# tanksha/das

Hardware: AMD Instinct MI355X
Metric: pattern matches/sec (bindings/s) + % HBM roofline (higher is better)
Workload: dtype u32; 1 GPU; config2 bio gene-level KB (+ annotation layouts): single-Link + 2-clause And (Q1-Q4) + scripts/benchmark.py QUERY_1-3 (Q3, Q5, Q6); parallelism=links sharded x1, step_calls=matched() per query

## Files before the change

das_amd/csrc/das_internal.h:

```cpp
#pragma once
#include <array>
#include <atomic>
#include <map>
#include <unordered_map>
#include <memory>
#include <mutex>
#include <string>
#include <vector>

#include "../../include/das_mi355x.h"
#include "common.h"
#include "prims.h"

namespace das {

constexpr int kMaxArity = 8;
constexpr int kMaxPosArity = 3;
constexpr int kMaxCols = 16;
constexpr int kTypeBits = 24;

enum AtomCat : uint8_t { CAT_OTHER = 0, CAT_NODE = 1, CAT_LINK = 2, CAT_LINK_REMOTE = 3 };
enum CatPrio : uint8_t { PRIO_OTHER = 0, PRIO_NODE = 1, PRIO_REMOTE = 2, PRIO_LINK = 3 };
__host__ __device__ inline uint8_t cat_of_prio(uint32_t p) {
  return p == PRIO_LINK ? CAT_LINK : p == PRIO_REMOTE ? CAT_LINK_REMOTE : p == PRIO_NODE ? CAT_NODE : CAT_OTHER;
// ... 46 lines not shown
struct Index {
  bool built = false;
  hipStream_t stream = nullptr;
  uint64_t n_atoms = 0, n_nodes = 0, n_links = 0, n_types = 0;
  uint32_t shard_world = 1;
  Digest* digest = nullptr;
  uint32_t* by_digest = nullptr;
  uint8_t* cat = nullptr;
  uint32_t* type = nullptr;
  uint32_t* arity = nullptr;
  uint64_t* tgt_off = nullptr;
  uint32_t* in_off = nullptr;
  uint32_t* in_link = nullptr;
  uint64_t in_total = 0;
  uint32_t* tgt = nullptr;
  uint32_t* ctype = nullptr;
  uint32_t* name_leaf = nullptr;
  std::array<RowTable, kMaxArity + 1> ttab{};
  std::array<RowTable, kMaxArity + 1> ctab{};
  std::array<std::array<PosIndex, kMaxPosArity>, kMaxPosArity + 1> pidx{};
  std::array<std::vector<uint64_t>, kMaxArity + 1> type_off;
  std::array<std::vector<uint32_t>, kMaxArity + 1> tbound, gbound;
  std::vector<Digest> ctype_digest;
  std::vector<Digest> type_digest;
  std::vector<uint8_t> no_pattern;
  bool no_pattern_any = false;
  bool blocked(uint32_t ty) const { return ty < no_pattern.size() && no_pattern[ty]; }
  std::vector<uint32_t> type_name_len;
  std::vector<CtypeRange> ctype_range;
  std::vector<Digest> h_node_dig;
  std::vector<uint32_t> h_node_id, h_node_type;
  NameHeap names;
  std::vector<void*> owned;
  std::map<std::array<uint64_t, 4>, std::pair<uint64_t, uint64_t>> range_cache;
  uint64_t device_bytes = 0;
};

struct Ctx;
struct Table;

struct Expansion;
struct ExpansionDel {
  void operator()(Expansion* e) const;
};

struct Lazy {
  enum Kind : uint8_t { PRODUCT = 0, VIEW = 1, EXPAND = 2 };
  Kind kind = PRODUCT;
  Ctx* ctx = nullptr;
  Table* owner = nullptr;
  std::atomic<bool> listed{false};
  std::unique_ptr<Expansion, ExpansionDel> exp;
  bool aliases_index() const { return kind != PRODUCT; }
  uint32_t* buf = nullptr;
  uint64_t np = 0, nb = 0, pcap = 0, bcap = 0;
  int ncp = 0, ncb = 0;
  int32_t pvars[kMaxCols] = {0}, bvars[kMaxCols] = {0};
  uint8_t side[kMaxCols] = {0}, src[kMaxCols] = {0};
  const uint32_t* pcol(int k) const { return buf + (uint64_t)k * pcap; }
  const uint32_t* bcol(int k) const { return buf + (uint64_t)ncp * pcap + (uint64_t)k * bcap; }
  Lazy() = default;
  Lazy(const Lazy&) = delete;
  Lazy& operator=(const Lazy&) = delete;
  ~Lazy() {
    if (buf) cache_free(buf);
  }
};

struct Table {
  int kind = DAS_TABLE_ORDERED;
  int ncols = 0;
  int sorted_col = -1;
  int32_t vars[kMaxCols] = {0};
  int32_t member[kMaxCols] = {0};
  uint32_t lo[kMaxCols] = {0};
  uint32_t hi[kMaxCols] = {kNone, kNone, kNone, kNone, kNone, kNone, kNone, kNone,
                           kNone, kNone, kNone, kNone, kNone, kNone, kNone, kNone};
  uint64_t nrows = 0, cap = 0;
  uint32_t* data = nullptr;
  hipStream_t s = nullptr;
  bool view = false;
  std::shared_ptr<Lazy> lazy;
  uint32_t* col(int c) const {
    DAS_CHECK(!lazy, DAS_E_INTERNAL, "column of an unresolved table");
    return data + (uint64_t)c * cap;
  }
  ~Table() {
    if (data && !view) cache_free(data);
  }
};

struct KStat {
  double ms = 0, bytes = 0;
  uint64_t launches = 0;
};
struct PendingEv {
  std::string name;
  hipEvent_t a, b;
  double bytes;
};

struct Ctx {
  bool prof = false;
  int scan_views = 0;
  std::string prof_only;
  std::string prof_tag;
  uint32_t tag_plan = ~0u;
  std::string tag_plan_name;
  hipStream_t gate_s = nullptr;
  double gate_min = 0;
  bool prof_selected(const std::string& name) const {
    if (prof_only.empty()) return true;
    size_t b = 0;
    while (b <= prof_only.size()) {
      size_t e = prof_only.find('|', b);
      if (e == std::string::npos) e = prof_only.size();
      if (prof_only.compare(b, e - b, name) == 0) return true;
      b = e + 1;
// ... 125 lines not shown
void partition_rows(Ctx& c, const uint32_t* d_rows, uint64_t n, uint32_t K, const uint8_t* d_owner, uint32_t world,
                    uint32_t* d_out, uint64_t* counts);
void numbered_strings(const char* prefix, uint64_t plen, uint64_t first, uint64_t n, uint8_t* out, uint64_t* off);
void synth_powerlaw_links(uint32_t* d_child, uint64_t first, uint64_t n, uint32_t K, uint32_t n_link_types,
                          uint32_t type_leaf0, uint32_t node_leaf0, uint64_t n_nodes, double s, uint64_t seed,
                          hipStream_t st);
void free_index(Ctx& c);
void lookup_digests(Ctx& c, const Digest* h_digests, uint64_t n, int64_t* h_ids);
bool lookup_small(Ctx& c, const Digest* h_digests, uint64_t n, int64_t* h_ids, uint8_t* cat, uint32_t* arity,
                  uint32_t* type);

void ensure_name_heap(Ctx& c);
void check_name_dfa(const das_name_dfa_t& d);
uint64_t match_node_names(Ctx& c, uint32_t type_id, const das_name_dfa_t& d, uint32_t* out_ids, uint64_t cap);
std::unique_ptr<struct Table> scan_node_names(Ctx& c, uint32_t type_id, const das_name_dfa_t& d, int32_t var);
std::unique_ptr<struct Table> table_name_filter(Ctx& c, const struct Table& t, int32_t var, uint32_t type_id,
                                                const das_name_dfa_t& d, int mode);
uint64_t node_names(Ctx& c, const uint32_t* h_ids, const uint32_t* d_ids, uint64_t n, uint64_t* off, uint8_t* bytes,
                    uint64_t cap, uint8_t* kind, uint64_t* n_other);

uint64_t atoms_json(Ctx& c, const uint32_t* h_ids, const uint32_t* d_ids, uint64_t n, uint32_t as_list,
                    const uint8_t* type_json, const uint64_t* type_json_off, uint32_t n_types, uint8_t* out,
                    uint64_t cap, uint64_t* n_other, uint64_t* n_bad_utf8);
uint64_t links_outgoing(Ctx& c, const uint32_t* h_ids, const uint32_t* d_ids, uint64_t n, uint64_t* off,
                        uint32_t* targets, uint64_t cap, uint32_t* ctype, uint8_t* kind);

void halo_expand(Ctx& c, const uint32_t* seed_ids, uint64_t n_seeds, uint32_t levels,
                 std::vector<std::unique_ptr<Table>>& links, std::vector<std::unique_ptr<Table>>& atoms);
std::unique_ptr<Table> pattern_counts(Ctx& c, const uint32_t* d_links, uint64_t n);
void conjunction_counts(Ctx& c, const uint32_t* tpl, uint64_t m, const uint32_t* combo, uint64_t n, uint32_t k,
                        uint64_t* counts);
void mine_combinations(Ctx& c, const uint32_t* tpl, uint64_t m, const uint64_t* tpl_count, const uint32_t* basics,
                       uint64_t nb, const uint32_t* cands, uint64_t nc, uint32_t k, uint64_t universe_size,
                       uint64_t support, bool normalized, uint32_t top, uint64_t max_combinations,
                       uint32_t* out_combo, uint64_t* out_count, double* out_value, uint32_t* n_out,
                       uint64_t stats[3]);

struct ColSet {
  const uint32_t* c[kMaxCols];
  int n;
};

ColSet cols_of(const Table& t);
void sort_perm(const ColSet& cs, uint64_t n, uint32_t* perm, int bits, hipStream_t s);
int id_bits(const Ctx& c);
std::unique_ptr<Table> gather_table(Ctx& c, const Table& a, const uint32_t* idx, uint64_t m);
std::unique_ptr<Table> gather_ranges(Ctx& c, const Table& a, const uint64_t* begin, const uint64_t* end,
                                     uint32_t n_ranges);
std::unique_ptr<Table> compact_table(Ctx& c, const Table& a, const uint32_t* keep);
void join_ranges(Ctx& c, const ColSet& probe, uint64_t np, const ColSet& build_sorted, uint64_t nb, uint32_t* lo,
                 uint32_t* cnt);
std::unique_ptr<Table> scan_link(Ctx& c, const das_link_scan_t& q);
std::unique_ptr<Table> scan_template(Ctx& c, const das_template_scan_t& q);
std::unique_ptr<Table> join(Ctx& c, const Table& a, const Table& b, int flags, bool defer_product = false);
void settle(Ctx& c, Table& t);
void register_alias(Table& t);
void deregister_alias(Lazy& r);
void settle_aliases(Ctx& c);
bool defer_join_rows(uint64_t probe_rows, uint64_t out_rows);
void make_lazy_view(Ctx& c, Table& t);
std::unique_ptr<Table> product_rows(Ctx& c, const Table& t, uint64_t row0, uint64_t n);
struct ExpansionCol {
  const uint32_t* key = nullptr;
  const uint32_t* rowid = nullptr;
  const uint2* lc = nullptr;
  uint64_t n = 0;
};
bool expansion_probe_col(const Table& t, int col, ExpansionCol& out);
void product_checksum(Ctx& c, const Table& t, const uint64_t* salt, uint64_t out[2]);
std::unique_ptr<Table> semi_join_multi(Ctx& c, const Table& p, const std::vector<const Table*>& qs);
std::unique_ptr<Table> index_join_filtered(Ctx& c, const Table& a, const das_link_scan_t& q, int32_t fvar,
                                           const std::vector<const Table*>& qs);
std::unique_ptr<Table> index_join(Ctx& c, const Table& a, const das_link_scan_t& q,
                                  std::unique_ptr<Table>* take = nullptr);
std::unique_ptr<Table> anti_index_join(Ctx& c, const Table& a, const das_link_scan_t& q);
std::unique_ptr<Table> antijoin(Ctx& c, const Table& a, const Table& t);
std::unique_ptr<Table> dedup(Ctx& c, const Table& a);
std::unique_ptr<Table> concat(Ctx& c, const Table* const* ts, int n);
std::unique_ptr<Table> new_table(Ctx& c, int kind, int ncols, const int32_t* vars, uint64_t cap,
                                 const int32_t* member = nullptr);
inline std::unique_ptr<Table> new_table_like(Ctx& c, const Table& a, uint64_t cap) {
  auto t = new_table(c, a.kind, a.ncols, a.vars, cap, a.member);
  t->sorted_col = a.sorted_col;
  for (int k = 0; k < a.ncols; ++k) {
    t->lo[k] = a.lo[k];
    t->hi[k] = a.hi[k];
  }
  return t;
}
std::unique_ptr<Table> partition(Ctx& c, const Table& t, const int32_t* key_vars, uint32_t nkey, uint32_t nparts,
                                 uint64_t* counts);
void export_rows(Ctx& c, const Table& t, uint32_t* dst);
void table_checksum(Ctx& c, const Table& t, const uint64_t* salt, uint64_t out[2]);
double box_store_bw(Ctx& c, uint64_t bytes, uint32_t reps);
void prof_mark(Ctx& c, uint32_t id);
std::unique_ptr<Table> import_rows(Ctx& c, int kind, int ncols, const int32_t* vars, const int32_t* member,
                                   const uint32_t* src, uint64_t n);

struct PlanOutput {
  bool matched = false, negation = false;
  std::vector<std::unique_ptr<Table>> tables;
};
PlanOutput plan_execute(Ctx& c, const das_plan_node_t* nodes, uint32_t n, int no_overload);
std::vector<PlanOutput> plan_execute_many(Ctx& c, const das_plan_node_t* const* nodes, const uint32_t* n,
                                          uint32_t n_plans, int no_overload);
PlanOutput plan_execute_sharded(Ctx& c, const das_plan_node_t* nodes, uint32_t n, int no_overload,
                                const std::vector<const Table*>& inputs, std::vector<uint8_t>& checks);
// ... 48 lines not shown
```

das_amd/csrc/plan.hip:

```cpp
#include <functional>
#include <memory>
#include <vector>

#include "das_internal.h"

namespace das {
namespace {

using TablePtr = std::unique_ptr<Table>;

struct Rel {
  std::vector<TablePtr> t;
  bool partial = false;
  bool nonempty() const {
    for (auto& x : t)
      if (x->nrows) return true;
    return false;
  }
  void push(TablePtr x) {
    if (x && x->nrows) t.push_back(std::move(x));
  }
};

struct Res {
// ... 26 lines not shown
  uint32_t next(uint32_t i) const {
    DAS_CHECK(i < n, DAS_E_INVALID, "plan: truncated node array");
    const das_plan_node_t& x = nd[i];
    if (x.op == DAS_PLAN_LINK || x.op == DAS_PLAN_CONST || x.op == DAS_PLAN_INPUT || x.op == DAS_PLAN_TEMPLATE)
      return i + 1;
    if (x.op == DAS_PLAN_NOT) return next(i + 1);
    DAS_CHECK(x.op == DAS_PLAN_AND || x.op == DAS_PLAN_OR || x.op == DAS_PLAN_TVM, DAS_E_INVALID,
              "plan: bad node op");
    uint32_t j = i + 1;
    for (uint32_t k = 0; k < x.nchild; ++k) j = next(j);
    return j;
  }

  std::vector<uint32_t> children(uint32_t i) const {
    std::vector<uint32_t> out;
    uint32_t j = i + 1;
    for (uint32_t k = 0; k < nd[i].nchild; ++k) {
      out.push_back(j);
      j = next(j);
    }
    return out;
  }

  Rel normalize(Rel a) {
    std::vector<std::vector<TablePtr>> groups;
    for (auto& x : a.t) {
      bool put = false;
      for (auto& g : groups)
        if (same_schema(*g[0], *x)) {
          g.push_back(std::move(x));
          put = true;
          break;
        }
      if (!put) {
        groups.emplace_back();
        groups.back().push_back(std::move(x));
      }
    }
    Rel out;
    out.partial = a.partial;
    for (auto& g : groups) {
      if (g.size() == 1) {
        out.push(std::move(g[0]));
        continue;
      }
      std::vector<const Table*> ts;
      for (auto& x : g) ts.push_back(x.get());
      auto cat = concat(c, ts.data(), (int)ts.size());
      out.push(dedup(c, *cat));
    }
    return out;
  }

  Rel join_rel(const Rel& a, const Rel& b, bool defer = false) {
    Rel out;
    out.partial = a.partial || b.partial;
    for (auto& ta : a.t)
      for (auto& tb : b.t) out.push(join(c, *ta, *tb, no_overload, defer && defer_rows(ta->nrows, tb->nrows)));
    return out;
  }

  static bool defer_rows(uint64_t na, uint64_t nb) {
    const char f = env_char("DAS_DEFER_PRODUCT");
    if (f == '0') return false;
    return f == '1' || na * nb > (1ull << 20);
  }

  void settle_for_normalize(Rel& acc) {
    for (size_t i = 0; i < acc.t.size(); ++i) {
      if (!acc.t[i]->lazy) continue;
      for (size_t j = 0; j < acc.t.size(); ++j)
        if (j != i && same_schema(*acc.t[i], *acc.t[j])) {
          settle(c, *acc.t[i]);
          break;
        }
    }
  }

  Rel antijoin_rel(Rel r, const Rel& f) {
    for (auto& ft : f.t) {
      Rel nx;
      nx.partial = r.partial;
      for (auto& t : r.t) nx.push(antijoin(c, *t, *ft));
      r = std::move(nx);
    }
    return r;
  }

  Rel minus_rel(Rel a, const Rel& b) {
    Rel out;
    out.partial = a.partial;
    for (auto& t : a.t) {
      TablePtr cur = std::move(t);
      for (auto& f : b.t)
        if (cur && cur->nrows && same_schema(*cur, *f)) cur = antijoin(c, *cur, *f);
      out.push(std::move(cur));
    }
    return out;
  }

  Res eval(uint32_t i) {
    const das_plan_node_t& x = nd[i];
    static const char* const kOp[] = {"?", "LINK", "CONST", "NOT", "AND", "OR", "INPUT", "TEMPLATE", "TVM"};
    if (trace_on()) trace_mark("node", x.op <= 8 ? kOp[x.op] : "?");
    Res r;
    switch (x.op) {
      case DAS_PLAN_CONST:
        r.matched = x.value != 0;
        return r;
      case DAS_PLAN_LINK: {
        DAS_CHECK(x.scan.ordered, DAS_E_UNSUPPORTED, "plan: unordered Link terms take the host path");
// ... 625 lines not shown
```

das_amd/csrc/query.hip:

```cpp
#include <algorithm>
#include <cstddef>
#include <cstdlib>
#include <cstring>
#include <optional>
#include <string>
#include <type_traits>

#include "das_internal.h"

namespace das {

namespace {

struct FlagIn {
  const uint32_t* a;
  uint64_t n;
  __device__ uint32_t operator()(uint64_t i) const { return i < n ? a[i] : 0u; }
};

struct WidenCnt {
  const uint32_t* a;
  uint64_t n;
  __device__ uint64_t operator()(uint64_t i) const { return i < n ? (uint64_t)a[i] : 0ull; }
};

constexpr unsigned B = 256;
constexpr int kChunkIters = 16;
constexpr uint64_t kChunk = (uint64_t)B * kChunkIters;
inline dim3 G(uint64_t n) { return dim3(grid_for(n, B)); }

struct ScanSpec {
  const uint32_t* col[kMaxArity + 1];
  uint32_t arity;
  uint32_t fixed[kMaxArity];
  int32_t outpos[kMaxCols];
  uint32_t nout;
  uint32_t eq_a[kMaxArity], eq_b[kMaxArity], neq;
  uint32_t no_overload;
  uint32_t unordered;
  uint32_t upos[kMaxArity], nupos;
  uint32_t emit_link;
  uint32_t all_keep;
};

__device__ __forceinline__ bool scan_keep(const ScanSpec& sp, uint64_t r) {
  if (sp.all_keep) return true;
  for (uint32_t p = 0; p < sp.arity; ++p)
    if (sp.fixed[p] != kNone && sp.col[1 + p][r] != sp.fixed[p]) return false;
  for (uint32_t e = 0; e < sp.neq; ++e)
    if (sp.col[1 + sp.eq_a[e]][r] != sp.col[1 + sp.eq_b[e]][r]) return false;
  if (sp.unordered) {
    for (uint32_t i = 0; i < sp.nupos; ++i)
      for (uint32_t j = i + 1; j < sp.nupos; ++j)
        if (sp.col[1 + sp.upos[i]][r] == sp.col[1 + sp.upos[j]][r]) return false;
  } else if (sp.no_overload) {
    const uint32_t base = sp.emit_link ? 1 : 0;
    for (uint32_t i = base; i < sp.nout; ++i)
      for (uint32_t j = i + 1; j < sp.nout; ++j)
        if (sp.col[1 + sp.outpos[i]][r] == sp.col[1 + sp.outpos[j]][r]) return false;
  }
  return true;
// ... 1382 lines not shown
std::unique_ptr<Table> gather_ranges(Ctx& c, const Table& a, const uint64_t* begin, const uint64_t* end,
                                     uint32_t n_ranges) {
  std::vector<uint64_t> h(2 * (uint64_t)n_ranges + 1, 0);
  uint64_t m = 0, last = 0;
  bool ascending = true;
  for (uint32_t i = 0; i < n_ranges; ++i) {
    DAS_CHECK(begin[i] <= end[i] && end[i] <= a.nrows, DAS_E_INVALID, "gather range outside the table");
    h[i] = m;
    h[n_ranges + 1 + i] = begin[i];
    m += end[i] - begin[i];
    if (end[i] > begin[i]) {
      if (begin[i] < last) ascending = false;
      last = end[i] - 1;
    }
  }
  h[n_ranges] = m;
  auto t = new_table_like(c, a, m);
  t->nrows = m;
  if (!ascending) t->sorted_col = -1;
  if (m && a.ncols) {
    DBuf<uint64_t> d(h.size(), c.s);
    DAS_HIP(hipMemcpyAsync(d.p, h.data(), 8 * h.size(), hipMemcpyHostToDevice, c.s));
    hipLaunchKernelGGL(k_gather_ranges, G(m), dim3(B), 0, c.s, cols_of(a), (const uint64_t*)d.p,
                       (const uint64_t*)d.p + n_ranges + 1, n_ranges, m, t->data, t->cap);
    DAS_HIP(hipGetLastError());
  }
  return t;
}

std::unique_ptr<Table> gather_table(Ctx& c, const Table& a, const uint32_t* idx, uint64_t m) {
  auto t = new_table_like(c, a, m);
  t->nrows = m;
  if (m && a.ncols) {
    hipLaunchKernelGGL(k_gather_cols, G(m), dim3(B), 0, c.s, cols_of(a), idx, m, t->data, t->cap);
    DAS_HIP(hipGetLastError());
  }
  return t;
}

template <typename Pred>
__device__ __forceinline__ uint32_t tile_flags(const Pred& pred, uint64_t base, uint64_t n) {
  bool f[kScanItems];
#pragma unroll
  for (int r = 0; r < kScanItems; ++r) {
    const uint64_t i = base + (uint64_t)r * kScanBlock + threadIdx.x;
    f[r] = pred(i < n ? i : n - 1) && i < n;
  }
  uint32_t bits = 0;
#pragma unroll
  for (int r = 0; r < kScanItems; ++r) bits |= (f[r] ? 1u : 0u) << r;
  return bits;
}

template <typename Pred>
__global__ void __launch_bounds__(kScanBlock) k_tile_count(Pred pred, uint64_t n, uint32_t* tcnt, uint8_t* fl) {
  static_assert(kScanItems <= 8, "one flag byte per thread");
  __shared__ uint32_t s[kScanBlock / 64];
  const uint64_t base = (uint64_t)blockIdx.x * kScanTile;
  const uint32_t bits = tile_flags(pred, base, n);
  fl[(uint64_t)blockIdx.x * kScanBlock + threadIdx.x] = (uint8_t)bits;
  uint32_t acc = __popc(bits);
  acc = wave_reduce_sum(acc);
  if (__lane_id() == 0) s[threadIdx.x >> 6] = acc;
  __syncthreads();
  if (threadIdx.x == 0) tcnt[blockIdx.x] = s[0] + s[1] + s[2] + s[3];
}

__global__ void __launch_bounds__(kScanBlock) k_compact_rows(const uint8_t* __restrict__ fl,
                                                             const uint32_t* __restrict__ toff, ColSet src,
                                                             uint32_t* __restrict__ out, uint64_t cap) {
  constexpr int W = kScanBlock / 64;
  __shared__ uint32_t s_wave[kScanItems][W];
  const uint64_t base = (uint64_t)blockIdx.x * kScanTile;
  const int wave = threadIdx.x >> 6;
  const uint32_t bits = fl[(uint64_t)blockIdx.x * kScanBlock + threadIdx.x];
  uint32_t inc[kScanItems];
#pragma unroll
  for (int r = 0; r < kScanItems; ++r) {
    inc[r] = wave_incl_sum_u32((bits >> r) & 1u);
    if (__lane_id() == 63) s_wave[r][wave] = inc[r];
  }
  __syncthreads();
  uint32_t carry = toff[blockIdx.x], o[kScanItems];
#pragma unroll
  for (int r = 0; r < kScanItems; ++r) {
    uint32_t pre = carry, all = 0;
#pragma unroll
    for (int w = 0; w < W; ++w) {
      pre += w < wave ? s_wave[r][w] : 0u;
      all += s_wave[r][w];
    }
    o[r] = pre + inc[r] - 1;
    carry += all;
  }
  for (int k = 0; k < src.n; ++k) {
    const uint32_t* col = src.c[k];
    uint32_t v[kScanItems];
#pragma unroll
    for (int r = 0; r < kScanItems; ++r)
      v[r] = ((bits >> r) & 1u) ? col[base + (uint64_t)r * kScanBlock + threadIdx.x] : 0u;
#pragma unroll
    for (int r = 0; r < kScanItems; ++r)
      if ((bits >> r) & 1u) out[(uint64_t)k * cap + o[r]] = v[r];
  }
}

struct FlagPred {
  const uint32_t* keep;
  __device__ __forceinline__ bool operator()(uint64_t i) const { return keep[i] != 0; }
};

template <typename Pred>
__global__ void __launch_bounds__(kSmallBlock) k_compact_small(Pred pred, uint64_t n, ColSet src, uint32_t* out,
                                                               uint64_t cap, uint32_t* slot, uint32_t seq,
                                                               const uint32_t* guard) {
  constexpr int W = kSmallBlock / 64;
  __shared__ uint32_t s_w[W];
  __shared__ uint32_t s_run;
  const int wave = threadIdx.x >> 6;
  const uint64_t lt = __lanemask_lt();
  if (guard && *guard) {
    if (threadIdx.x == 0) publish_u32(slot, seq, 0xFFFFFFFFu);
    return;
  }
  if (threadIdx.x == 0) s_run = 0;
  __syncthreads();
  for (uint64_t r0 = 0; r0 < n; r0 += kSmallBlock) {
    const uint64_t r = r0 + threadIdx.x;
    const bool keep = r < n && pred(r);
    const uint64_t m = __ballot(keep);
    if (__lane_id() == 0) s_w[wave] = __popcll(m);
    __syncthreads();
    uint32_t pos = s_run + __popcll(m & lt);
    for (int w = 0; w < wave; ++w) pos += s_w[w];
    if (keep)
      for (int k = 0; k < src.n; ++k) out[(uint64_t)k * cap + pos] = src.c[k][r];
    __syncthreads();
    if (threadIdx.x == 0) {
      uint32_t t = 0;
      for (int w = 0; w < W; ++w) t += s_w[w];
      s_run += t;
    }
    __syncthreads();
  }
  if (threadIdx.x == 0) publish_u32(slot, seq, s_run);
}

__global__ void k_guard_count(uint32_t* tcnt, const uint32_t* guard) {
  if (threadIdx.x == 0 && *guard) tcnt[0] |= 0x80000000u;
}

template <typename Pred>
std::unique_ptr<Table> compact_pred(Ctx& c, const Table& a, Pred pred, const char* prof = nullptr,
                                    double pred_bytes = 4.0, const uint32_t* guard = nullptr) {
  const uint64_t n = a.nrows;
  if (!n) return gather_table(c, a, nullptr, 0);
  const bool fused_guard = !env_is("DAS_SMALL_GUARD", '0');
  if (guard && (n >= (1ull << 31) || (n <= kSmallScan && !fused_guard))) {
    if (read_u32(guard, c.s)) return nullptr;
    guard = nullptr;
  }
  if (n <= kSmallScan) {
    auto t = new_table_like(c, a, n);
    const PubSlot ps = pub_reserve();
    hipLaunchKernelGGL((k_compact_small<Pred>), dim3(1), dim3(kSmallBlock), 0, c.s, pred, n, cols_of(a), t->data,
                       t->cap, ps.p, ps.seq, guard);
    DAS_HIP(hipGetLastError());
    uint32_t m = 0;
    pub_wait(ps, c.s, &m, 1);
    if (m == 0xFFFFFFFFu) return nullptr;
    t->nrows = m;
    return t;
  }
  const uint64_t tiles = (n + kScanTile - 1) / kScanTile;
  DAS_CHECK(tiles < (1ull << 31), DAS_E_UNSUPPORTED, "compaction: too many rows");
  DBuf<uint32_t> tcnt(tiles, c.s), toff(tiles + 1, c.s);
  DBuf<uint8_t> fl(tiles * kScanBlock, c.s);
  {
    std::optional<ProfScope> ps;
    if (prof) ps.emplace(c, prof, pred_bytes * n);
    hipLaunchKernelGGL((k_tile_count<Pred>), dim3((unsigned)tiles), dim3(kScanBlock), 0, c.s, pred, n, tcnt.p, fl.p);
    DAS_HIP(hipGetLastError());
  }
  if (guard) {
    hipLaunchKernelGGL(k_guard_count, dim3(1), dim3(64), 0, c.s, tcnt.p, guard);
    DAS_HIP(hipGetLastError());
  }
  uint64_t mx = 0;
  const uint64_t m = scan_total<uint32_t>(SpanIn<uint32_t>{tcnt.p}, tiles, toff.p, c.s, &mx);
  if (guard && mx >= 0x80000000ull) return nullptr;
  auto t = new_table_like(c, a, m);
  t->nrows = m;
  if (m && a.ncols) {
    std::optional<ProfScope> ps;
    if (prof) ps.emplace(c, "k_compact_rows", n / 8.0 + 8.0 * a.ncols * m);
    hipLaunchKernelGGL(k_compact_rows, dim3((unsigned)tiles), dim3(kScanBlock), 0, c.s, (const uint8_t*)fl.p,
                       (const uint32_t*)toff.p, cols_of(a), t->data, t->cap);
    DAS_HIP(hipGetLastError());
  }
  return t;
}

std::unique_ptr<Table> compact_table(Ctx& c, const Table& a, const uint32_t* keep) {
  return compact_pred(c, a, FlagPred{keep});
}

void join_ranges(Ctx& c, const ColSet& probe, uint64_t np, const ColSet& build_sorted, uint64_t nb, uint32_t* lo,
                 uint32_t* cnt) {
  if (!np) return;
  hipLaunchKernelGGL(k_join_count, G(np), dim3(B), 0, c.s, probe, np, build_sorted, nb, lo, cnt);
  DAS_HIP(hipGetLastError());
}

std::unique_ptr<Table> new_table(Ctx& c, int kind, int ncols, const int32_t* vars, uint64_t cap,
                                 const int32_t* member) {
  DAS_CHECK(ncols >= 0 && ncols <= kMaxCols, DAS_E_UNSUPPORTED, "too many columns in a binding table");
  auto t = std::make_unique<Table>();
  t->kind = kind;
  t->ncols = ncols;
  for (int i = 0; i < ncols; ++i) t->vars[i] = vars ? vars[i] : 0;
  for (int i = 0; i < ncols; ++i) t->member[i] = member ? member[i] : -1;
  for (int i = 0; i < ncols; ++i) {
    t->lo[i] = 0;
    t->hi[i] = kNone;
  }
  t->s = c.s;
  t->cap = col_stride(cap ? cap : 1);
  if (ncols) t->data = (uint32_t*)cache_alloc(4ull * ncols * t->cap, c.s);
  return t;
}

namespace {

std::unique_ptr<Table> run_scan_rows(Ctx& c, ScanSpec& sp, uint64_t begin, uint64_t end, int kind, int ncols,
                                     const int32_t* vars);

void scan_bounds(const Index& idx, const ScanSpec& sp, uint32_t type_id, Table& t) {
  const uint32_t ar = sp.arity, ncol = ar + 1;
  auto src = [&](int col, uint32_t& lo, uint32_t& hi) {
    const auto& tb = idx.tbound[ar];
    const auto& gb = idx.gbound[ar];
    if (type_id != kNone && (uint64_t)(type_id + 1) * ncol * 2 <= tb.size()) {
      lo = tb[((uint64_t)type_id * ncol + col) * 2];
// ... 2358 lines not shown
    res->nrows = w[1];
    out = std::move(res);
  }
  return 1;
}

__global__ void k_bits_set(const uint32_t* __restrict__ key, uint64_t n, uint32_t kmin, uint32_t range,
                           uint32_t* bits, uint32_t* dup) {
  uint32_t d = 0;
  for (uint64_t i = blockIdx.x * (uint64_t)blockDim.x + threadIdx.x; i < n; i += (uint64_t)gridDim.x * blockDim.x) {
    const uint32_t k = key[i] - kmin;
    if (k >= range) continue;
    const uint32_t m = 1u << (k & 31);
    if (atomicOr(&bits[k >> 5], m) & m) d = 1;
  }
  if (__ballot(d) && __lane_id() == 0) atomicOr(dup, 1u);
}
__global__ void k_bits_set_sorted(const uint32_t* __restrict__ key, uint64_t n, uint32_t kmin, uint32_t range,
                                  uint32_t* bits, uint32_t* dup) {
  const int lane = __lane_id();
  uint32_t d = 0;
  const uint64_t stride = (uint64_t)gridDim.x * blockDim.x;
  for (uint64_t i0 = blockIdx.x * (uint64_t)blockDim.x; i0 < n; i0 += stride) {
    const uint64_t i = i0 + threadIdx.x;
    const uint32_t k = i < n ? key[i] - kmin : 0xFFFFFFFFu;
    const bool act = k < range;
    const uint32_t w = act ? k >> 5 : 0xFFFFFFFFu;
    uint32_t m = act ? 1u << (k & 31) : 0u;
#pragma unroll
    for (int st = 1; st < 64; st <<= 1) {
      const uint32_t om = (uint32_t)__shfl_up(m, st, 64), ow = (uint32_t)__shfl_up(w, st, 64);
      if (lane >= st && ow == w && act) {
        if (om & (1u << (k & 31))) d = 1;
        m |= om;
      }
    }
    const uint32_t nw = (uint32_t)__shfl_down(w, 1, 64);
    const bool tail = act && (lane == 63 || nw != w);
    if (tail && (atomicOr(&bits[w], m) & m)) d = 1;
  }
  if (__ballot(d) && __lane_id() == 0) atomicOr(dup, 1u);
}

struct BitsPred {
  const uint32_t* key;
  uint32_t kmin, range;
  const uint32_t* bits;
  __device__ __forceinline__ bool operator()(uint64_t i) const {
    const uint32_t k = key[i] - kmin;
    return k < range && ((bits[k >> 5] >> (k & 31)) & 1u);
  }
};

std::unique_ptr<Table> semi_join(Ctx& c, const Table& P, const Table& Q) {
  if (env_is("DAS_SEMI_JOIN", '0')) return nullptr;
  const int32_t var = Q.vars[0];
  int pk = -1;
  for (int i = 0; i < P.ncols; ++i) if (P.vars[i] == var) pk = i;
  if (pk < 0 || Q.nrows >= 0xFFFFFFFFull) return nullptr;
  uint32_t lo = Q.lo[0], hi = Q.hi[0];
  if (hi == kNone || lo > hi) {
    lo = 0;
    hi = (uint32_t)(c.idx.n_atoms ? c.idx.n_atoms - 1 : 0);
  }
  const uint64_t range = (uint64_t)hi - lo + 1;
  if (range > (1ull << 31)) return nullptr;
  const uint64_t words = (range + 31) / 32;
  DBuf<uint32_t> bits(words + 1, c.s);
  fill_dev(bits.p, 0, 4 * (words + 1), c.s);
  {
    ProfScope ps(c, "join_build", 4.0 * Q.nrows + 4.0 * words);
    hipLaunchKernelGGL(k_bits_set, G(Q.nrows), dim3(B), 0, c.s, (const uint32_t*)Q.col(0), Q.nrows, lo, (uint32_t)range,
                       bits.p, bits.p + words);
    DAS_HIP(hipGetLastError());
  }
  return compact_pred(c, P, BitsPred{(const uint32_t*)P.col(pk), lo, (uint32_t)range, (const uint32_t*)bits.p},
                      "k_tile_count<BitsPred>", 4.0, (const uint32_t*)bits.p + words);
}

__global__ void k_bits_and(uint32_t* __restrict__ acc, const uint32_t* __restrict__ b, uint64_t words) {
  for (uint64_t i = blockIdx.x * (uint64_t)blockDim.x + threadIdx.x; i < words; i += (uint64_t)gridDim.x * blockDim.x)
    acc[i] &= b[i];
}

bool key_bits(Ctx& c, const std::vector<const Table*>& Qs, int32_t var, uint64_t& lo, uint64_t& hi,
              DBuf<uint32_t>& acc) {
  auto clip = [&](uint32_t l, uint32_t h) {
    if (h == kNone || l > h) return;
    lo = std::max<uint64_t>(lo, l);
    hi = std::min<uint64_t>(hi, h);
  };
  for (const Table* Q : Qs) {
    if (Q->kind != DAS_TABLE_ORDERED || Q->ncols != 1 || Q->vars[0] != var || Q->nrows >= 0xFFFFFFFFull) return false;
    clip(Q->lo[0], Q->hi[0]);
  }
  if (lo > hi) return true;
  const uint64_t range = hi - lo + 1;
  if (range > (1ull << 31)) return false;
  const uint64_t words = (range + 31) / 32;
  acc.alloc(words + 1, c.s);
  DBuf<uint32_t> one(Qs.size() > 1 ? words + 1 : 1, c.s);
  for (size_t i = 0; i < Qs.size(); ++i) {
    uint32_t* bits = i == 0 ? acc.p : one.p;
    fill_dev(bits, 0, 4 * (i == 0 ? words + 1 : words), c.s);
    {
      ProfScope ps(c, "join_build", 4.0 * Qs[i]->nrows + 4.0 * words);
      if (Qs[i]->sorted_col == 0)
        hipLaunchKernelGGL(k_bits_set_sorted, G(Qs[i]->nrows), dim3(B), 0, c.s, (const uint32_t*)Qs[i]->col(0),
                           Qs[i]->nrows, (uint32_t)lo, (uint32_t)range, bits, acc.p + words);
      else
        hipLaunchKernelGGL(k_bits_set, G(Qs[i]->nrows), dim3(B), 0, c.s, (const uint32_t*)Qs[i]->col(0),
                           Qs[i]->nrows, (uint32_t)lo, (uint32_t)range, bits, acc.p + words);
      DAS_HIP(hipGetLastError());
    }
    if (i) {
      KScope ks("k_bits_and", 12.0 * words);
      hipLaunchKernelGGL(k_bits_and, G(words), dim3(B), 0, c.s, acc.p, (const uint32_t*)one.p, words);
      DAS_HIP(hipGetLastError());
    }
// ... 153 lines not shown
        hipLaunchKernelGGL(k_chunk_compact<kStageChunk>, dim3(sgrid), dim3(B), 0, c.s, (const uint32_t*)scr.p, scap,
                           (const uint32_t*)ccnt.p, (const uint32_t*)coff.p, 0ull, nch, nu, out->data, out->cap);
      else
        hipLaunchKernelGGL(k_chunk_compact<(int)kBalChunk>, dim3(sgrid), dim3(B), 0, c.s, (const uint32_t*)scr.p, scap,
                           (const uint32_t*)ccnt.p, (const uint32_t*)coff.p, 0ull, nch, nu, out->data, out->cap);
      DAS_HIP(hipGetLastError());
    }
    return finish(std::move(out));
  }
  const uint64_t chunks = (total + kBalChunk - 1) / kBalChunk;
  const unsigned fgrid = grid_for(chunks, B / 64, 65535u * 4u);
  DBuf<uint8_t> fl(total, c.s);
  DBuf<uint32_t> ccnt(chunks, c.s), coff(chunks + 1, c.s);
  {
    ProfScope ps(c, "k_dj_filt<0,-1,-1>", 12.0 * A.nrows + 5.0 * total);
    hipLaunchKernelGGL((k_dj_filt<0, -1, -1>), dim3(fgrid), dim3(B), 0, c.s, rows, A.nrows, 0u, nrows, lcp, units, offp,
                       total, fk, fl.p, ccnt.p, (const uint32_t*)nullptr, jc, (uint32_t*)nullptr, 0ull, 0ull, chunks);
    DAS_HIP(hipGetLastError());
  }
  const uint64_t m = scan_total<uint32_t>(SpanIn<uint32_t>{ccnt.p}, chunks, coff.p, c.s);
  auto out = new_table(c, DAS_TABLE_ORDERED, nu, pl.uni.data(), m);
  out->nrows = m;
  if (m) {
    ProfScope ps(c, "k_dj_filt<1," + targs,
                 (12.0 + 4.0 * jc.np) * A.nrows + 1.0 * total + 4.0 * jc.nb * m + 4.0 * nu * m);
    with_shape([&](auto NP, auto NB) {
      hipLaunchKernelGGL((k_dj_filt<1, NP(), NB()>), dim3(fgrid), dim3(B), 0, c.s, rows, A.nrows, 0u, nrows, lcp, units,
                         offp, total, fk, fl.p, (uint32_t*)nullptr, (const uint32_t*)coff.p, jc, out->data, out->cap,
                         0ull, chunks);
    });
  }
  return finish(std::move(out));
}

namespace {
void launch_cartesian(Ctx& c, const OutMap& om, uint64_t np, uint64_t nb, uint64_t first, uint64_t n, Table& out) {
  const int nu = om.n;
  ProfScope ps(c, "k_cartesian<" + std::to_string(nu >= 2 && nu <= 6 ? nu : 0) + ">", 4.0 * nu * n);
  const unsigned cg = grid_for((n + 3) / 4, B);
  const uint64_t S = 4ull * cg * B, sq = S / nb, sr = S % nb;
  DAS_CHECK(out.cap % 4 == 0 && out.cap >= ((n + 3) & ~3ull) && (reinterpret_cast<uintptr_t>(out.data) & 15) == 0,
            DAS_E_INTERNAL, "cartesian: output columns not 16-byte aligned");
  switch (nu) {
    case 2: hipLaunchKernelGGL(k_cartesian<2>, dim3(cg), dim3(B), 0, c.s, om, np, nb, first, n, sq, sr, out.data, out.cap); break;
    case 3: hipLaunchKernelGGL(k_cartesian<3>, dim3(cg), dim3(B), 0, c.s, om, np, nb, first, n, sq, sr, out.data, out.cap); break;
    case 4: hipLaunchKernelGGL(k_cartesian<4>, dim3(cg), dim3(B), 0, c.s, om, np, nb, first, n, sq, sr, out.data, out.cap); break;
    case 5: hipLaunchKernelGGL(k_cartesian<5>, dim3(cg), dim3(B), 0, c.s, om, np, nb, first, n, sq, sr, out.data, out.cap); break;
    case 6: hipLaunchKernelGGL(k_cartesian<6>, dim3(cg), dim3(B), 0, c.s, om, np, nb, first, n, sq, sr, out.data, out.cap); break;
    default: hipLaunchKernelGGL(k_cartesian<0>, dim3(cg), dim3(B), 0, c.s, om, np, nb, first, n, sq, sr, out.data, out.cap); break;
  }
  DAS_HIP(hipGetLastError());
}

OutMap product_map(const Table& t) {
  const Lazy& r = *t.lazy;
  OutMap om{};
  om.n = t.ncols;
  for (int k = 0; k < t.ncols; ++k) {
    om.side[k] = r.side[k];
    om.col[k] = r.side[k] ? r.bcol(r.src[k]) : r.pcol(r.src[k]);
  }
  return om;
}

Table factor_view(const Table& t, int side) {
  const Lazy& r = *t.lazy;
  Table f;
  f.kind = DAS_TABLE_ORDERED;
  f.ncols = side ? r.ncb : r.ncp;
  for (int k = 0; k < f.ncols; ++k) f.vars[k] = side ? r.bvars[k] : r.pvars[k];
  f.nrows = side ? r.nb : r.np;
  f.cap = side ? r.bcap : r.pcap;
  f.data = const_cast<uint32_t*>(side ? r.bcol(0) : r.pcol(0));
  f.s = t.s;
  f.view = true;
  return f;
}
}

void register_alias(Table& t) {
  if (!t.lazy || !t.lazy->aliases_index() || t.lazy->owner) return;
  t.lazy->owner = &t;
  t.lazy->ctx->aliases.push_back(t.lazy.get());
  t.lazy->listed.store(true, std::memory_order_release);
}

void deregister_alias(Lazy& r) {
  if (!r.owner) return;
  auto& v = r.ctx->aliases;
  v.erase(std::remove(v.begin(), v.end(), &r), v.end());
  r.owner = nullptr;
  r.listed.store(false, std::memory_order_release);
}

void settle_aliases(Ctx& c) {
  while (!c.aliases.empty()) settle(c, *c.aliases.back()->owner);
}

void make_lazy_view(Ctx& c, Table& t) {
  DAS_CHECK(t.view && !t.lazy, DAS_E_INTERNAL, "make_lazy_view: not a view");
  auto r = std::make_shared<Lazy>();
  r->kind = Lazy::VIEW;
  r->ctx = &c;
  t.lazy = std::move(r);
}

// ... 3 lines not shown
  const uint64_t cap = col_stride(t.nrows ? t.nrows : 1);
  uint32_t* data = (uint32_t*)cache_alloc(4ull * t.ncols * cap, c.s);
  deregister_alias(*r);
  if (r->kind == Lazy::PRODUCT) {
    const OutMap om = product_map(t);
    t.lazy.reset();
    t.data = data;
    t.cap = cap;
    t.s = c.s;
    launch_cartesian(c, om, r->np, r->nb, 0, t.nrows, t);
    return;
  }
  if (r->kind == Lazy::VIEW) {
    const uint32_t* src = t.data;
    const uint64_t ld = t.cap;
    for (int k = 0; k < t.ncols; ++k) copy_dev(data + (uint64_t)k * cap, src + (uint64_t)k * ld, 4 * t.nrows, c.s);
    t.lazy.reset();
    t.view = false;
    t.data = data;
    t.cap = cap;
    t.s = c.s;
    return;
  }
  const Expansion& e = *r->exp;
  t.lazy.reset();
  t.data = data;
  t.cap = cap;
  t.s = c.s;
  dj_write_rows(c, e.probe->nrows, e.probe->ncols, e.rowid.p, 0u, e.probe->nrows, e.lc.p, e.k, e.jc, e.nu,
                -4.0 * e.jc.nb, data, cap);
}

std::unique_ptr<Table> product_rows(Ctx& c, const Table& t, uint64_t row0, uint64_t n) {
  DAS_CHECK(t.lazy && t.lazy->kind == Lazy::PRODUCT, DAS_E_INTERNAL, "product_rows: not a deferred product");
  DAS_CHECK(row0 <= t.nrows && n <= t.nrows - row0, DAS_E_INVALID, "rows out of range");
  auto out = new_table(c, DAS_TABLE_ORDERED, t.ncols, t.vars, n);
  out->nrows = n;
  if (n) launch_cartesian(c, product_map(t), t.lazy->np, t.lazy->nb, row0, n, *out);
  return out;
}

void product_checksum(Ctx& c, const Table& t, const uint64_t* salt, uint64_t out[2]) {
  DAS_CHECK(t.lazy && t.lazy->kind == Lazy::PRODUCT, DAS_E_INTERNAL, "product_checksum: not a deferred product");
  const Lazy& r = *t.lazy;
  uint64_t sp[kMaxCols] = {0}, sb[kMaxCols] = {0};
  for (int k = 0; k < t.ncols; ++k) (r.side[k] ? sb : sp)[r.src[k]] = salt[k];
  uint64_t hp[2], hb[2];
  table_checksum(c, factor_view(t, 0), sp, hp);
  table_checksum(c, factor_view(t, 1), sb, hb);
  out[0] = hp[0] * hb[0];
  out[1] = hp[1] * r.nb + hb[1] * r.np;
}

std::unique_ptr<Table> join(Ctx& c, const Table& A, const Table& Bt, int no_overload, bool defer_product) {
  if (A.kind != DAS_TABLE_ORDERED || Bt.kind != DAS_TABLE_ORDERED) return theta_join(c, A, Bt, no_overload);
  std::vector<int32_t> va(A.vars, A.vars + A.ncols), vb(Bt.vars, Bt.vars + Bt.ncols), shared, uni;
  std::set_intersection(va.begin(), va.end(), vb.begin(), vb.end(), std::back_inserter(shared));
  std::set_union(va.begin(), va.end(), vb.begin(), vb.end(), std::back_inserter(uni));
  DAS_CHECK((int)uni.size() <= kMaxCols, DAS_E_UNSUPPORTED, "too many variables");
  auto colof = [](const Table& t, int32_t v) {
    for (int i = 0; i < t.ncols; ++i) if (t.vars[i] == v) return i;
    return -1;
  };
  const int nu = (int)uni.size();
  if (A.nrows == 0 || Bt.nrows == 0) return new_table(c, DAS_TABLE_ORDERED, nu, uni.data(), 0);
  const bool a_probe = A.nrows >= Bt.nrows;
  const Table& P = a_probe ? A : Bt;
  const Table& Q = a_probe ? Bt : A;
  std::unique_ptr<Table> out;
  if (shared.empty() && defer_product && !no_overload && P.ncols && Q.ncols) {
    const uint64_t total = P.nrows * Q.nrows;
    out = std::make_unique<Table>();
    out->ncols = nu;
    for (int k = 0; k < nu; ++k) {
      out->vars[k] = uni[k];
      out->member[k] = -1;
    }
    out->s = c.s;
    out->nrows = total;
    auto r = std::make_shared<Lazy>();
    r->ctx = &c;
    r->np = P.nrows;
    r->nb = Q.nrows;
    r->ncp = P.ncols;
    r->ncb = Q.ncols;
    r->pcap = col_stride(P.nrows);
    r->bcap = col_stride(Q.nrows);
    r->buf = (uint32_t*)cache_alloc(4ull * (r->ncp * r->pcap + r->ncb * r->bcap), c.s);
    for (int k = 0; k < P.ncols; ++k) {
      r->pvars[k] = P.vars[k];
      copy_dev(const_cast<uint32_t*>(r->pcol(k)), P.col(k), 4 * P.nrows, c.s);
    }
    for (int k = 0; k < Q.ncols; ++k) {
      r->bvars[k] = Q.vars[k];
      copy_dev(const_cast<uint32_t*>(r->bcol(k)), Q.col(k), 4 * Q.nrows, c.s);
    }
    for (int k = 0; k < nu; ++k) {
      const int ip = colof(P, uni[k]);
      r->side[k] = ip >= 0 ? 0 : 1;
      r->src[k] = (uint8_t)(ip >= 0 ? ip : colof(Q, uni[k]));
    }
    out->lazy = std::move(r);
  } else if (shared.empty()) {
    const uint64_t total = P.nrows * Q.nrows;
    out = new_table(c, DAS_TABLE_ORDERED, nu, uni.data(), total);
    out->nrows = total;
    OutMap om{};
    om.n = nu;
    for (int k = 0; k < nu; ++k) {
      int ip = colof(P, uni[k]);
      if (ip >= 0) { om.col[k] = P.col(ip); om.side[k] = 0; }
      else { om.col[k] = Q.col(colof(Q, uni[k])); om.side[k] = 1; }
    }
    launch_cartesian(c, om, P.nrows, Q.nrows, 0, total, *out);
  } else if (shared.size() == 1 && Q.ncols == 1 && (out = semi_join(c, P, Q))) {
  } else if (shared.size() == 1 && (out = direct_join(c, P, Q, shared[0], uni))) {
  } else {
    ColSet qk{};
    qk.n = (int)shared.size();
    for (int k = 0; k < qk.n; ++k) qk.c[k] = Q.col(colof(Q, shared[k]));
    DBuf<uint32_t> perm(Q.nrows, c.s);
    {
      ProfScope ps(c, "join_build_sort", 4.0 * Q.nrows * (Q.ncols + 2));
      sort_perm(qk, Q.nrows, perm.p, id_bits(c), c.s);
    }
    auto Qs = gather_table(c, Q, perm.p, Q.nrows);
    perm.release();
    ColSet qks{}, pk{};
    qks.n = pk.n = (int)shared.size();
    for (int k = 0; k < qks.n; ++k) {
      qks.c[k] = Qs->col(colof(*Qs, shared[k]));
      pk.c[k] = P.col(colof(P, shared[k]));
    }
    DBuf<uint32_t> lo(P.nrows, c.s), cnt(P.nrows, c.s);
    DBuf<uint64_t> offs(P.nrows + 1, c.s);
    {
      ProfScope ps(c, "k_join_count", 4.0 * P.nrows * (pk.n + 2));
      hipLaunchKernelGGL(k_join_count, G(P.nrows), dim3(B), 0, c.s, pk, P.nrows, qks, Qs->nrows, lo.p, cnt.p);
      DAS_HIP(hipGetLastError());
    }
    const uint64_t total = scan_total<uint64_t>(WidenCnt{cnt.p, P.nrows}, P.nrows, offs.p, c.s);
    out = new_table(c, DAS_TABLE_ORDERED, nu, uni.data(), total);
    out->nrows = total;
    if (total) {
      OutMap om{};
      om.n = nu;
      for (int k = 0; k < nu; ++k) {
        int ip = colof(P, uni[k]);
// ... 226 lines not shown
```

Baseline: 734.7 billion bindings/s.

## Add LDS keyset semi-join, fused tile-count publish, and zero-copy product factors

Adds an LDS hash keyset predicate for semi-joins with small key sets, so each block builds the set in shared memory instead of filling a global bitmap. Fuses the tile count, guard check and prefix scan into one kernel whose last block publishes the totals to the host, removing separate scan and guard launches. Deferred cartesian products now take ownership of input table buffers when possible, or copy all columns in one kernel, instead of issuing a copy per column. Each block rebuilds the hash set redundantly, and taking ownership empties the source tables, which changes their lifetime assumptions.

```diff
diff --git a/das_amd/csrc/das_internal.h b/das_amd/csrc/das_internal.h
--- a/das_amd/csrc/das_internal.h
+++ b/das_amd/csrc/das_internal.h
@@ -122,18 +122,24 @@
   std::atomic<bool> listed{false};
   std::unique_ptr<Expansion, ExpansionDel> exp;
   bool aliases_index() const { return kind != PRODUCT; }
+  uint32_t* pown = nullptr;
+  uint32_t* bown = nullptr;
   uint32_t* buf = nullptr;
+  const uint32_t* pbase = nullptr;
+  const uint32_t* bbase = nullptr;
   uint64_t np = 0, nb = 0, pcap = 0, bcap = 0;
   int ncp = 0, ncb = 0;
   int32_t pvars[kMaxCols] = {0}, bvars[kMaxCols] = {0};
   uint8_t side[kMaxCols] = {0}, src[kMaxCols] = {0};
-  const uint32_t* pcol(int k) const { return buf + (uint64_t)k * pcap; }
-  const uint32_t* bcol(int k) const { return buf + (uint64_t)ncp * pcap + (uint64_t)k * bcap; }
+  const uint32_t* pcol(int k) const { return pbase + (uint64_t)k * pcap; }
+  const uint32_t* bcol(int k) const { return bbase + (uint64_t)k * bcap; }
   Lazy() = default;
   Lazy(const Lazy&) = delete;
   Lazy& operator=(const Lazy&) = delete;
   ~Lazy() {
     if (buf) cache_free(buf);
+    if (pown) cache_free(pown);
+    if (bown) cache_free(bown);
   }
 };
 
@@ -365,7 +371,8 @@
                  uint32_t* cnt);
 std::unique_ptr<Table> scan_link(Ctx& c, const das_link_scan_t& q);
 std::unique_ptr<Table> scan_template(Ctx& c, const das_template_scan_t& q);
-std::unique_ptr<Table> join(Ctx& c, const Table& a, const Table& b, int flags, bool defer_product = false);
+std::unique_ptr<Table> join(Ctx& c, const Table& a, const Table& b, int flags, bool defer_product = false,
+                            std::unique_ptr<Table>* take_a = nullptr, std::unique_ptr<Table>* take_b = nullptr);
 void settle(Ctx& c, Table& t);
 void register_alias(Table& t);
 void deregister_alias(Lazy& r);
diff --git a/das_amd/csrc/keyset.h b/das_amd/csrc/keyset.h
--- /dev/null
+++ b/das_amd/csrc/keyset.h
@@ -0,0 +1,49 @@
+#pragma once
+#include <cstdint>
+
+#if defined(__HIPCC__) || defined(__CUDACC__)
+#define DAS_KS_HD __host__ __device__ __forceinline__
+#else
+#define DAS_KS_HD inline
+#endif
+
+namespace das {
+
+constexpr uint32_t kKeySetMax = 2048;
+constexpr uint32_t kKeySetMaxSlots = 2 * kKeySetMax;
+constexpr uint32_t kKeySetMinSlots = 64;
+constexpr uint32_t kKeySetEmpty = 0xFFFFFFFFu;
+
+DAS_KS_HD uint32_t ks_log2_slots(uint32_t n) {
+  uint32_t lg = 6;
+  while ((1u << lg) < 2 * n && (1u << lg) < kKeySetMaxSlots) ++lg;
+  return lg;
+}
+
+DAS_KS_HD uint32_t ks_slot(uint32_t key, uint32_t lg) { return (key * 2654435769u) >> (32 - lg); }
+DAS_KS_HD uint32_t ks_next(uint32_t slot, uint32_t lg) { return (slot + 1) & ((1u << lg) - 1); }
+
+template <typename Cas>
+DAS_KS_HD uint32_t ks_insert(Cas cas, uint32_t key, uint32_t lg) {
+  uint32_t s = ks_slot(key, lg);
+  for (uint32_t step = 0; step < (1u << lg); ++step) {
+    const uint32_t old = cas(s, kKeySetEmpty, key);
+    if (old == kKeySetEmpty) return 0;
+    if (old == key) return 1;
+    s = ks_next(s, lg);
+  }
+  return 0;
+}
+
+DAS_KS_HD bool ks_contains(const uint32_t* set, uint32_t key, uint32_t lg) {
+  uint32_t s = ks_slot(key, lg);
+  for (uint32_t step = 0; step < (1u << lg); ++step) {
+    const uint32_t v = set[s];
+    if (v == key) return true;
+    if (v == kKeySetEmpty) return false;
+    s = ks_next(s, lg);
+  }
+  return false;
+}
+
+}
diff --git a/das_amd/csrc/plan.hip b/das_amd/csrc/plan.hip
--- a/das_amd/csrc/plan.hip
+++ b/das_amd/csrc/plan.hip
@@ -102,11 +102,14 @@
     return out;
   }
 
-  Rel join_rel(const Rel& a, const Rel& b, bool defer = false) {
+  Rel join_rel(Rel& a, Rel& b, bool defer = false) {
     Rel out;
     out.partial = a.partial || b.partial;
+    const bool take = defer && a.t.size() == 1 && b.t.size() == 1;
     for (auto& ta : a.t)
-      for (auto& tb : b.t) out.push(join(c, *ta, *tb, no_overload, defer && defer_rows(ta->nrows, tb->nrows)));
+      for (auto& tb : b.t)
+        out.push(join(c, *ta, *tb, no_overload, defer && defer_rows(ta->nrows, tb->nrows), take ? &ta : nullptr,
+                      take ? &tb : nullptr));
     return out;
   }
 
diff --git a/das_amd/csrc/query.hip b/das_amd/csrc/query.hip
--- a/das_amd/csrc/query.hip
+++ b/das_amd/csrc/query.hip
@@ -7,6 +7,7 @@
 #include <type_traits>
 
 #include "das_internal.h"
+#include "keyset.h"
 
 namespace das {
 
@@ -1495,18 +1496,76 @@
   return bits;
 }
 
+template <typename Pred, typename = void>
+struct pred_lds : std::false_type {};
 template <typename Pred>
-__global__ void __launch_bounds__(kScanBlock) k_tile_count(Pred pred, uint64_t n, uint32_t* tcnt, uint8_t* fl) {
+struct pred_lds<Pred, std::void_t<decltype(Pred::kLdsSlots)>> : std::true_type {};
+template <typename Pred>
+constexpr uint32_t pred_lds_slots() {
+  if constexpr (pred_lds<Pred>::value) return Pred::kLdsSlots;
+  else return 1;
+}
+template <typename Pred>
+struct LdsBound {
+  const Pred& p;
+  const uint32_t* lds;
+  __device__ __forceinline__ bool operator()(uint64_t i) const { return p.test(lds, i); }
+};
+
+template <typename Pred>
+__device__ __forceinline__ uint32_t tile_count_body(const Pred& pred, uint64_t n, uint8_t* fl, uint32_t* s_lds,
+                                                    uint32_t* s) {
   static_assert(kScanItems <= 8, "one flag byte per thread");
-  __shared__ uint32_t s[kScanBlock / 64];
   const uint64_t base = (uint64_t)blockIdx.x * kScanTile;
-  const uint32_t bits = tile_flags(pred, base, n);
+  uint32_t bits, mark = 0;
+  if constexpr (pred_lds<Pred>::value) {
+    mark = pred.build(s_lds) && blockIdx.x == 0 ? 0x80000000u : 0u;
+    bits = tile_flags(LdsBound<Pred>{pred, s_lds}, base, n);
+  } else {
+    bits = tile_flags(pred, base, n);
+  }
   fl[(uint64_t)blockIdx.x * kScanBlock + threadIdx.x] = (uint8_t)bits;
   uint32_t acc = __popc(bits);
   acc = wave_reduce_sum(acc);
   if (__lane_id() == 0) s[threadIdx.x >> 6] = acc;
   __syncthreads();
-  if (threadIdx.x == 0) tcnt[blockIdx.x] = s[0] + s[1] + s[2] + s[3];
+  return (s[0] + s[1] + s[2] + s[3]) | mark;
+}
+
+template <typename Pred>
+__global__ void __launch_bounds__(kScanBlock) k_tile_count(Pred pred, uint64_t n, uint32_t* tcnt, uint8_t* fl) {
+  __shared__ uint32_t s[kScanBlock / 64];
+  __shared__ uint32_t s_lds[pred_lds_slots<Pred>()];
+  const uint32_t cnt = tile_count_body(pred, n, fl, s_lds, s);
+  if (threadIdx.x == 0) tcnt[blockIdx.x] = cnt;
+}
+
+template <typename Pred>
+__global__ void __launch_bounds__(kScanBlock) k_tile_count_pub(Pred pred, uint64_t n, uint32_t* tcnt, uint8_t* fl,
+                                                               uint64_t tiles, uint32_t* toff,
+                                                               const uint32_t* guard, unsigned long long* ctr,
+                                                               unsigned long long last, uint32_t* slot,
+                                                               uint32_t seq) {
+  __shared__ uint32_t s[kScanBlock / 64];
+  __shared__ uint32_t s_lds[pred_lds_slots<Pred>()];
+  __shared__ uint64_t s_mx[kScanBlock / 64];
+  __shared__ int s_last;
+  const uint32_t cnt = tile_count_body(pred, n, fl, s_lds, s);
+  if (threadIdx.x == 0) {
+    __hip_atomic_store(&tcnt[blockIdx.x], cnt, __ATOMIC_RELAXED, __HIP_MEMORY_SCOPE_AGENT);
+    asm volatile("s_waitcnt vmcnt(0)" ::: "memory");
+    s_last = __hip_atomic_fetch_add(ctr, 1ull, __ATOMIC_RELAXED, __HIP_MEMORY_SCOPE_AGENT) == last;
+  }
+  __syncthreads();
+  if (!s_last) return;
+  __builtin_amdgcn_fence(__ATOMIC_ACQUIRE, "agent");
+  uint32_t total;
+  uint64_t mx;
+  block_scan_loop<uint32_t>(SpanIn<uint32_t>{tcnt}, tiles, toff, total, mx, s, s_mx);
+  if (threadIdx.x == 0) toff[tiles] = total;
+  if (guard && *guard) mx |= 0x80000000ull;
+  const uint32_t w[4] = {total, 0u, (uint32_t)mx, (uint32_t)(mx >> 32)};
+  pub_store(slot, seq, w, 4);
 }
 
 __global__ void __launch_bounds__(kScanBlock) k_compact_rows(const uint8_t* __restrict__ fl,
@@ -1560,9 +1619,12 @@
   constexpr int W = kSmallBlock / 64;
   __shared__ uint32_t s_w[W];
   __shared__ uint32_t s_run;
+  __shared__ uint32_t s_lds[pred_lds_slots<Pred>()];
   const int wave = threadIdx.x >> 6;
   const uint64_t lt = __lanemask_lt();
-  if (guard && *guard) {
+  bool voided = guard && *guard;
+  if constexpr (pred_lds<Pred>::value) voided = pred.build(s_lds) || voided;
+  if (voided) {
     if (threadIdx.x == 0) publish_u32(slot, seq, 0xFFFFFFFFu);
     return;
   }
@@ -1570,7 +1632,9 @@
   __syncthreads();
   for (uint64_t r0 = 0; r0 < n; r0 += kSmallBlock) {
     const uint64_t r = r0 + threadIdx.x;
-    const bool keep = r < n && pred(r);
+    bool keep;
+    if constexpr (pred_lds<Pred>::value) keep = r < n && pred.test(s_lds, r);
+    else keep = r < n && pred(r);
     const uint64_t m = __ballot(keep);
     if (__lane_id() == 0) s_w[wave] = __popcll(m);
     __syncthreads();
@@ -1619,19 +1683,39 @@
   DAS_CHECK(tiles < (1ull << 31), DAS_E_UNSUPPORTED, "compaction: too many rows");
   DBuf<uint32_t> tcnt(tiles, c.s), toff(tiles + 1, c.s);
   DBuf<uint8_t> fl(tiles * kScanBlock, c.s);
-  {
-    std::optional<ProfScope> ps;
-    if (prof) ps.emplace(c, prof, pred_bytes * n);
-    hipLaunchKernelGGL((k_tile_count<Pred>), dim3((unsigned)tiles), dim3(kScanBlock), 0, c.s, pred, n, tcnt.p, fl.p);
-    DAS_HIP(hipGetLastError());
-  }
-  if (guard) {
-    hipLaunchKernelGGL(k_guard_count, dim3(1), dim3(64), 0, c.s, tcnt.p, guard);
-    DAS_HIP(hipGetLastError());
-  }
-  uint64_t mx = 0;
-  const uint64_t m = scan_total<uint32_t>(SpanIn<uint32_t>{tcnt.p}, tiles, toff.p, c.s, &mx);
-  if (guard && mx >= 0x80000000ull) return nullptr;
+  const bool pub = tiles <= kCountPubUnits && !env_is("DAS_TILE_PUB", '0');
+  uint64_t m = 0, mx = 0;
+  if (pub) {
+    ScanCtr& ct = scan_ctr(c.s);
+    const PubSlot slot = pub_reserve();
+    {
+      std::optional<ProfScope> ps;
+      if (prof) ps.emplace(c, prof, pred_bytes * n);
+      hipLaunchKernelGGL((k_tile_count_pub<Pred>), dim3((unsigned)tiles), dim3(kScanBlock), 0, c.s, pred, n, tcnt.p,
+                         fl.p, tiles, toff.p, guard, ct.p, (unsigned long long)(ct.base + tiles - 1), slot.p,
+                         slot.seq);
+      DAS_HIP(hipGetLastError());
+      ct.base += tiles;
+    }
+    uint32_t w[4];
+    pub_wait(slot, c.s, w, 4);
+    m = (uint64_t)w[0] | ((uint64_t)w[1] << 32);
+    mx = (uint64_t)w[2] | ((uint64_t)w[3] << 32);
+  } else {
+    {
+      std::optional<ProfScope> ps;
+      if (prof) ps.emplace(c, prof, pred_bytes * n);
+      hipLaunchKernelGGL((k_tile_count<Pred>), dim3((unsigned)tiles), dim3(kScanBlock), 0, c.s, pred, n, tcnt.p,
+                         fl.p);
+      DAS_HIP(hipGetLastError());
+    }
+    if (guard) {
+      hipLaunchKernelGGL(k_guard_count, dim3(1), dim3(64), 0, c.s, tcnt.p, guard);
+      DAS_HIP(hipGetLastError());
+    }
+    m = scan_total<uint32_t>(SpanIn<uint32_t>{tcnt.p}, tiles, toff.p, c.s, &mx);
+  }
+  if ((guard || pred_lds<Pred>::value) && mx >= 0x80000000ull) return nullptr;
   auto t = new_table_like(c, a, m);
   t->nrows = m;
   if (m && a.ncols) {
@@ -4096,6 +4180,32 @@
   }
 };
 
+struct KeySetPred {
+  static constexpr uint32_t kLdsSlots = kKeySetMaxSlots;
+  const uint32_t* key;
+  const uint32_t* qkey;
+  uint32_t nq, kmin, range, lg;
+  __device__ __forceinline__ bool build(uint32_t* set) const {
+    __shared__ uint32_t s_dup;
+    if (threadIdx.x == 0) s_dup = 0;
+    for (uint32_t i = threadIdx.x; i < (1u << lg); i += blockDim.x) set[i] = kKeySetEmpty;
+    __syncthreads();
+    uint32_t d = 0;
+    for (uint32_t i = threadIdx.x; i < nq; i += blockDim.x) {
+      const uint32_t k = qkey[i] - kmin;
+      if (k >= range) continue;
+      d |= ks_insert([set](uint32_t s, uint32_t expect, uint32_t v) { return atomicCAS(&set[s], expect, v); }, k, lg);
+    }
+    if (d) s_dup = 1;
+    __syncthreads();
+    return s_dup != 0;
+  }
+  __device__ __forceinline__ bool test(const uint32_t* set, uint64_t i) const {
+    const uint32_t k = key[i] - kmin;
+    return k < range && ks_contains(set, k, lg);
+  }
+};
+
 std::unique_ptr<Table> semi_join(Ctx& c, const Table& P, const Table& Q) {
   if (env_is("DAS_SEMI_JOIN", '0')) return nullptr;
   const int32_t var = Q.vars[0];
@@ -4109,6 +4219,11 @@
   }
   const uint64_t range = (uint64_t)hi - lo + 1;
   if (range > (1ull << 31)) return nullptr;
+  if (Q.nrows && Q.nrows <= kKeySetMax && !env_is("DAS_SEMI_KEYSET", '0'))
+    return compact_pred(c, P,
+                        KeySetPred{(const uint32_t*)P.col(pk), (const uint32_t*)Q.col(0), (uint32_t)Q.nrows, lo,
+                                   (uint32_t)range, ks_log2_slots((uint32_t)Q.nrows)},
+                        "k_tile_count<KeySetPred>", 4.0);
   const uint64_t words = (range + 31) / 32;
   DBuf<uint32_t> bits(words + 1, c.s);
   fill_dev(bits.p, 0, 4 * (words + 1), c.s);
@@ -4368,6 +4483,30 @@
   DAS_HIP(hipGetLastError());
 }
 
+__global__ void k_copy_cols(ColSet src, uint64_t n, uint32_t* __restrict__ dst, uint64_t cap) {
+  const uint64_t total = n * (uint64_t)src.n;
+  for (uint64_t i = blockIdx.x * (uint64_t)blockDim.x + threadIdx.x; i < total; i += (uint64_t)gridDim.x * blockDim.x) {
+    const uint64_t k = i / n, r = i - k * n;
+    dst[k * cap + r] = src.c[k][r];
+  }
+}
+
+void product_factor(Ctx& c, const Table& t, std::unique_ptr<Table>* take, uint32_t*& own, uint64_t& cap) {
+  if (take && take->get() == &t && !t.view && !t.lazy && t.data) {
+    Table& mine = **take;
+    own = mine.data;
+    cap = mine.cap;
+    mine.data = nullptr;
+    mine.cap = 0;
+    return;
+  }
+  cap = col_stride(t.nrows);
+  own = (uint32_t*)cache_alloc(4ull * t.ncols * cap, c.s);
+  KScope ks("k_copy_cols", 8.0 * t.ncols * t.nrows);
+  hipLaunchKernelGGL(k_copy_cols, G(t.nrows * (uint64_t)t.ncols), dim3(B), 0, c.s, cols_of(t), t.nrows, own, cap);
+  DAS_HIP(hipGetLastError());
+}
+
 OutMap product_map(const Table& t) {
   const Lazy& r = *t.lazy;
   OutMap om{};
@@ -4477,7 +4616,8 @@
   out[1] = hp[1] * r.nb + hb[1] * r.np;
 }
 
-std::unique_ptr<Table> join(Ctx& c, const Table& A, const Table& Bt, int no_overload, bool defer_product) {
+std::unique_ptr<Table> join(Ctx& c, const Table& A, const Table& Bt, int no_overload, bool defer_product,
+                            std::unique_ptr<Table>* take_a, std::unique_ptr<Table>* take_b) {
   if (A.kind != DAS_TABLE_ORDERED || Bt.kind != DAS_TABLE_ORDERED) return theta_join(c, A, Bt, no_overload);
   std::vector<int32_t> va(A.vars, A.vars + A.ncols), vb(Bt.vars, Bt.vars + Bt.ncols), shared, uni;
   std::set_intersection(va.begin(), va.end(), vb.begin(), vb.end(), std::back_inserter(shared));
@@ -4509,16 +4649,22 @@
     r->nb = Q.nrows;
     r->ncp = P.ncols;
     r->ncb = Q.ncols;
-    r->pcap = col_stride(P.nrows);
-    r->bcap = col_stride(Q.nrows);
-    r->buf = (uint32_t*)cache_alloc(4ull * (r->ncp * r->pcap + r->ncb * r->bcap), c.s);
-    for (int k = 0; k < P.ncols; ++k) {
-      r->pvars[k] = P.vars[k];
-      copy_dev(const_cast<uint32_t*>(r->pcol(k)), P.col(k), 4 * P.nrows, c.s);
-    }
-    for (int k = 0; k < Q.ncols; ++k) {
-      r->bvars[k] = Q.vars[k];
-      copy_dev(const_cast<uint32_t*>(r->bcol(k)), Q.col(k), 4 * Q.nrows, c.s);
+    for (int k = 0; k < P.ncols; ++k) r->pvars[k] = P.vars[k];
+    for (int k = 0; k < Q.ncols; ++k) r->bvars[k] = Q.vars[k];
+    if (env_is("DAS_PRODUCT_TAKE", '0')) {
+      r->pcap = col_stride(P.nrows);
+      r->bcap = col_stride(Q.nrows);
+      r->buf = (uint32_t*)cache_alloc(4ull * (r->ncp * r->pcap + r->ncb * r->bcap), c.s);
+      r->pbase = r->buf;
+      r->bbase = r->buf + (uint64_t)r->ncp * r->pcap;
+      for (int k = 0; k < P.ncols; ++k) copy_dev(const_cast<uint32_t*>(r->pcol(k)), P.col(k), 4 * P.nrows, c.s);
+      for (int k = 0; k < Q.ncols; ++k) copy_dev(const_cast<uint32_t*>(r->bcol(k)), Q.col(k), 4 * Q.nrows, c.s);
+    } else {
+      if (&A == &Bt) take_a = take_b = nullptr;
+      product_factor(c, P, a_probe ? take_a : take_b, r->pown, r->pcap);
+      product_factor(c, Q, a_probe ? take_b : take_a, r->bown, r->bcap);
+      r->pbase = r->pown;
+      r->bbase = r->bown;
     }
     for (int k = 0; k < nu; ++k) {
       const int ip = colof(P, uni[k]);
```

Result: faster. 875.2 billion bindings/s (median of 5 runs) (+19.1%).
